# ArnaudPel/CamKifu

Hardware: AMD Instinct MI355X
Metric: frames/sec on 1920x1080 video + 19x19 stone-grid match % vs reference SGF (higher is better)
Workload: dtype u8+f16x2(f32 accumulate); 1 GPU; 1920x1080 synthetic game film, 256-frame batches resident in HBM, K1-K12 per ...; cnn=f16x2, frames_per_gpu=256, height=1080, width=1920, parallelism=frames of one video dealt x1, lanes_per_gpu=2, batches_in_flight=2

## Files before the change

### camkifu_amd/capi.py

```python
import ctypes as C
import os
import subprocess

import numpy as np

_HERE = os.path.dirname(os.path.abspath(__file__))
SO_PATH = os.environ.get("CK_HIP_LIB") or os.path.join(_HERE, "libck_hip.so")
CSRC = os.path.join(_HERE, "csrc")

CK_HOST, CK_DEVICE = 0, 1
CK_CNN_FP32, CK_CNN_BF16, CK_CNN_F16X2, CK_CNN_F16Q8 = 0, 1, 2, 3
CK_CNN_DEFAULT = CK_CNN_F16X2
CK_BOARD_LINES, CK_BOARD_NO_CONTOUR, CK_BOARD_TOO_SMALL = 0, 1, 2

ZONE_LINES = 32

EXPORTS = [
    "ck_ctx_create", "ck_ctx_create_prio", "ck_ctx_destroy", "ck_ctx_destroy2", "ck_stream_wait", "ck_last_error", "ck_backend", "ck_version", "ck_stream",
    "ck_timing_enable", "ck_timing_reset", "ck_timing_get",
    "ck_median15", "ck_median", "ck_canny", "ck_goban_canny", "ck_board_edges", "ck_board_lines", "ck_board_detect",
    "ck_i420_to_bgr", "ck_pyr_down", "ck_i420_to_bgr_pyr", "ck_get_perspective_transform", "ck_warp_perspective",
    "ck_mog2_create", "ck_mog2_apply", "ck_mog2_destroy", "ck_mog2_get_state",
    "ck_cnn_set_weights", "ck_cnn_set_mode", "ck_cnn_predict", "ck_cnn_maps", "ck_stones_detect",
    "ck_train_create", "ck_train_destroy", "ck_train_step", "ck_train_grads", "ck_train_apply", "ck_train_get_weights",
    "ck_train_get_adam_state", "ck_train_handover",
    "ck_cnn_regions", "ck_stones_run", "ck_zone_counts", "ck_mog2_band_run",
    "ck_board_detect_records", "ck_cnn_regions_records",
    "ck_contour_stones", "ck_cluster_stones", "ck_rng_get", "ck_rng_set", "ck_contours_external", "ck_find_intersections", "ck_update_grid",
    "ck_ordered_hull", "ck_boardfold_create", "ck_boardfold_destroy", "ck_boardfold_reset", "ck_boardfold_step", "ck_boardfold_run", "ck_round10", "ck_round10_reference",
    "ck_policy_create", "ck_policy_destroy", "ck_policy_run", "ck_policy_run_records", "ck_policy_get_state", "ck_policy_set_state",
    "ck_policy_watch",
]

WEIGHT_ORDER = ("c1w", "c1b", "c2w", "c2b", "c3w", "c3b", "c4w", "c4b", "d1w", "d1b", "d2w", "d2b")
WEIGHT_SHAPES = dict(c1w=(5, 5, 3, 32), c1b=(32,), c2w=(5, 5, 32, 32), c2b=(32,),
                     c3w=(3, 3, 32, 90), c3b=(90,), c4w=(3, 3, 90, 90), c4b=(90,),
                     d1w=(3240, 160), d1b=(160,), d2w=(160, 81), d2b=(81,))

# ... 64 lines not shown
        L.ck_policy_set_state.argtypes = [C.c_void_p, C.c_void_p, C.c_int]
        L.ck_policy_watch.argtypes = [C.c_void_p, C.c_int, C.c_int, C.c_int, C.c_double, C.c_longlong]
        L.ck_cluster_stones.argtypes = ([C.c_void_p, C.c_void_p, C.c_int, C.c_int, C.c_int, C.c_int, C.c_void_p, C.c_void_p, C.c_void_p,
                                        C.c_int] + [C.c_void_p] * 5 + [C.c_longlong] + [C.c_void_p] * 3)
        L.ck_rng_get.argtypes = [C.c_void_p, C.c_void_p]
        L.ck_train_step.argtypes = ([C.c_void_p, C.c_int, C.c_void_p, C.c_void_p] + [C.c_int] * 5
                                    + [C.c_double, C.c_int, C.c_uint64, C.c_void_p])
        L.ck_train_grads.argtypes = ([C.c_void_p, C.c_int, C.c_void_p, C.c_void_p] + [C.c_int] * 5
                                     + [C.c_int, C.c_uint64, C.c_longlong] + [C.c_void_p] * 5)
        L.ck_train_apply.argtypes = [C.c_void_p, C.c_int, C.c_void_p, C.c_double]
        L.ck_rng_set.argtypes = [C.c_void_p, C.c_uint64]
        _lib = L
    return _lib


def _is_torch(a):
    return type(a).__module__.startswith("torch")


def pyr_shape(h, w, levels):
    h, w, levels = int(h), int(w), int(levels)
    if levels < 0:
        raise CkError("pyramid levels %d: negative" % levels)
    for l in range(levels):
        if h < 2 or w < 2:
            raise CkError("pyramid level %d would take a %dx%d image: sides below 2" % (l + 1, w, h))
        h, w = (h + 1) // 2, (w + 1) // 2
    return h, w


# ... 265 lines not shown
    def cnn_set_weights(self, weights):
        ptrs = (C.c_void_p * 12)()
        keep, space = [], None
        for i, k in enumerate(WEIGHT_ORDER):
            a = weights[k]
            assert tuple(a.shape) == WEIGHT_SHAPES[k], (k, tuple(a.shape))
            if _is_torch(a):
                import torch
                assert a.dtype == torch.float32
            p, sp, ka = self._in(a, np.float32)
            assert space in (None, sp), "weights must live in one memory space"
            space = sp
            ptrs[i] = p
            keep.append(ka)
        self._chk(lib().ck_cnn_set_weights(self._h, ptrs, space))

    def cnn_set_mode(self, mode):
        self._chk(lib().ck_cnn_set_mode(self._h, int(mode)))

    def cnn_predict(self, goban, want_y=True):
        shp = tuple(goban.shape)
        n = 1 if len(shp) == 3 else shp[0]
        p, sp, keep = self._in(goban)
        y, yp = None, None
        if want_y:
            y, yp, _ = self._out(goban, (n, 100, 81), np.float32)
        labels, lp, osp = self._out(goban, (n, 19, 19), np.uint8)
        conf, cp, _ = self._out(goban, (n, 19, 19), np.float64)
        self._chk(lib().ck_cnn_predict(self._h, p, n, sp, yp, lp, cp, osp))
        return (y, labels, conf) if want_y else (labels, conf)
# ... 452 lines not shown
```

### camkifu_amd/csrc/ck_api.hip

```cpp
#include <stdarg.h>
#include <stddef.h>

#include <cfloat>
#include <cmath>
#include <algorithm>
#include <vector>
#include <thread>
#include <chrono>

#include "ck_common.h"
#include "ck_stonegeom.h"

thread_local std::string g_ck_create_error;
static thread_local const ck_ctx* g_ck_busy_ctx = nullptr;

unsigned long long ck_thread_token()
{
    static std::atomic<unsigned long long> next{1};
    static thread_local unsigned long long mine = 0;
    if (!mine) mine = next.fetch_add(1);
    return mine;
}
void ck_note_busy(const ck_ctx* ctx) { g_ck_busy_ctx = ctx; }

// ... 551 lines not shown
    return finish(ctx);
    CK_API_END(ctx)
}

int ck_cnn_set_weights(ck_ctx* ctx, const float* const weights[12], int space)
{
    CK_API_BEGIN(ctx)
    if (!ctx || !weights) return CK_ERR_ARG;
    for (int i = 0; i < 12; i++) if (!weights[i]) return ck_fail(ctx, CK_ERR_ARG, "weights[%d] is NULL", i);
    CK_HIP(ctx, hipSetDevice(ctx->device));
    CK_TRY(k_cnn_pack_weights(ctx, weights, space));
    return finish(ctx);
    CK_API_END(ctx)
}

int ck_cnn_set_mode(ck_ctx* ctx, int mode)
{
    CK_API_BEGIN(ctx)
    if (!ctx) return CK_ERR_ARG;
    if (mode != CK_CNN_FP32 && mode != CK_CNN_BF16 && mode != CK_CNN_F16X2 && mode != CK_CNN_F16Q8) return ck_fail(ctx, CK_ERR_ARG, "unknown cnn mode %d", mode);
    ctx->cnn_mode = mode;
    return CK_OK;
    CK_API_END(ctx)
}

struct RegionOut { uint8_t* label = nullptr; double* conf = nullptr; ck_frame_record* rec = nullptr; int rec_space = CK_HOST; };

static int ensure_rec_host(ck_ctx* ctx, size_t bytes)
{
    if (bytes <= ctx->rec_host_cap) return CK_OK;
// ... 620 lines not shown
```

### camkifu_amd/csrc/ck_common.h

```cpp
#pragma once
#include <hip/hip_runtime.h>
#include <stdint.h>
#include <stdio.h>
#include <string.h>
#include <atomic>
#include <condition_variable>
#include <functional>
#include <memory>
#include <mutex>
#include <exception>
#include <map>
#include <stdexcept>
#include <string>
#include <thread>
#include <vector>

#include "../../include/camkifu_amd.h"

struct DevBuf {
    void* p = nullptr;
    size_t cap = 0;
};

struct TimingSlot {
// ... 24 lines not shown
    long long steps = 0;
    DevBuf w, g, m, v;
    DevBuf lab, a1, a2, p1, a3, a4, p2, h1, lg, dlg, dh1, dp2, dz4, dz3, dp1, dz2, dz1, part, lossv, mask1, mask2, mask3;
};

static inline bool ck_cnn_split(int mode) { return mode == CK_CNN_F16X2 || mode == CK_CNN_F16Q8; }

struct CnnWeights {
    bool set = false;
    DevBuf c1w, c1b, c2w, c2b, c3w, c3b, c4w, c4b, d1w, d1b, d2w, d2b;
    DevBuf c2w_bf, c3w_bf, c4w_bf, d1w_bf;
    DevBuf c1w_f16;
    DevBuf d1w_bfp;
    DevBuf c1w_h2, c2w_h2, c3w_h2, c4w_h2, d1w_h2;
    DevBuf c1w_q8, c2x_q8, c3x_q8, c4x_q8;
    bool q8_ok = false;
};

struct ck_ctx {
    std::atomic<unsigned long long> owner{0};
    int depth = 0;
    int device = 0;
    hipStream_t stream = nullptr;
    std::string err;
    bool timing = false;
    std::map<std::string, TimingSlot> slots;
    std::vector<PendingEvent> pending;
    std::vector<hipEvent_t> event_pool;
    hipEvent_t handover = nullptr;

// ... 20 lines not shown
    DevBuf out_stage;
    DevBuf mats;
    DevBuf pyr0, pyr1;
    void* host_pinned = nullptr;
    size_t host_pinned_cap = 0;
    void* host_pinned2 = nullptr;
    size_t host_pinned2_cap = 0;
    void* rec_host = nullptr;
    size_t rec_host_cap = 0;
    DevBuf rec_stage;

    CnnWeights cnn;
    int* cnn_flag_host = nullptr;
    int* cnn_flag_dev = nullptr;
    int cnn_fallbacks = 0;
    int cnn_mode = CK_CNN_F16X2;
    std::vector<Mog2State> mog2;
    std::vector<CkTrainer> trainers;
    uint64_t rng_state = 0xffffffffULL;
};

extern thread_local std::string g_ck_create_error;

int ck_fail(ck_ctx* ctx, int code, const char* fmt, ...);
int ck_ensure(ck_ctx* ctx, DevBuf& b, size_t bytes);
int ck_ensure_pinned(ck_ctx* ctx, size_t bytes, int which = 0);

#define CK_HIP(ctx, call)                                                                 \
    do {                                                                                  \
        hipError_t e__ = (call);                                                          \
// ... 92 lines not shown
    std::vector<int32_t> pts;
};
int k_contour_survey(ck_ctx* ctx, const uint8_t* d_edges, int n, int h, int w, std::vector<std::vector<CkContour>>& out);
int ck_goban_canny_dev(ck_ctx* ctx, const uint8_t* d_in, int n, int h, int w, uint8_t* d_edges, double* otsu_out);
int k_contour_stones(ck_ctx* ctx, const uint8_t* d_goban, const uint8_t* d_fg, int n, int side, const int32_t* rects,
                     int rs, int re, int cs, int ce, uint8_t* stones, int16_t* zones_out, uint8_t* mask_out);
int k_cluster_stones(ck_ctx* ctx, const void* d_imgs, int n, int side, int is_f32, const int32_t* rects, const uint8_t* mask,
                     const int32_t* jobs, int m, uint8_t* stones, uint8_t* trusted, uint8_t* ratios, float* centers,
                     uint8_t* labels, long long labels_cap, int32_t* passes, double* compact, int32_t* winner);
double ck_otsu_level(const int* hist, size_t npx);
int k_grid_lines(ck_ctx* ctx, const uint8_t* d_goban, int n, int side, const int32_t* rects, const int16_t** lines_out,
                 const int32_t** nlines_out, uint8_t* edges_out);
int k_cnn_predict(ck_ctx* ctx, const uint8_t* d_goban, int n, float* d_y, uint8_t* d_labels, double* d_conf,
                  int* d_nonfinite = nullptr, uint8_t* d_rlabel = nullptr, double* d_rconf = nullptr);
int k_cnn_pack_weights(ck_ctx* ctx, const float* const w[12], int space);
int k_cnn_bf16_pack_conv1(ck_ctx* ctx, const float* k1, DevBuf& dst);
int k_cnn_bf16_convs(ck_ctx* ctx, const uint8_t* gob, int np, uint16_t* p2, uint16_t* q4);
int k_cnn_bf16_pack_fc1(ck_ctx* ctx, const float* w, DevBuf& dst);
int k_cnn_bf16_fc1(ck_ctx* ctx, const uint16_t* q4, int np, float* h1);
int k_cnn_q8_pack(ck_ctx* ctx, const float* k1, const float* k2, const float* k3, const float* k4);
int k_cnn_q8_conv12(ck_ctx* ctx, const uint8_t* gob, int np, float* p2, int* overflow);
int k_cnn_q8_conv34(ck_ctx* ctx, const float* p2, int np, float* p4, int* overflow);
extern const size_t CK_TRAIN_COUNTS[12];
size_t ck_train_offset(int i);
int k_train_create(ck_ctx* ctx, CkTrainer& tr, const float* const w[12], int space);
void k_train_free(CkTrainer& tr);
int k_train_grads(ck_ctx* ctx, CkTrainer& tr, const uint8_t* d_x, const uint8_t* d_lab, int n, int drop, uint64_t seed,
                  uint64_t step, bool want_masks);
int k_train_adam(ck_ctx* ctx, CkTrainer& tr, const float* d_g, double lr);
int k_mog2_apply(ck_ctx* ctx, Mog2State& st, const uint8_t* d_img, double lr, uint8_t* d_fg);
// ... 11 lines not shown
```

### camkifu_amd/csrc/k_cnn.hip

```cpp
#include <math.h>

#include <algorithm>

#include <type_traits>

#include "ck_common.h"

#ifndef C3_WM
#define C3_WM 2
#endif
#ifndef C4_WM
#define C4_WM 2
#endif
#ifndef H2_STAGE_UNROLL
#define H2_STAGE_UNROLL 8
#endif
#ifndef H2C2S_PF
#define H2C2S_PF 1
#endif
#ifndef H2C2S_SB
#define H2C2S_SB true
#endif
#ifndef H2C3_PF
#define H2C3_PF 2
// ... 36 lines not shown
__device__ unsigned long long g_h2_prof[8];
__device__ unsigned long long g_h34_prof[8];
constexpr int H2_LOG_CAP = 1 << 18;
__device__ unsigned long long g_h2_log[3 * H2_LOG_CAP];
#define H34_STAMP(K) do { if (NXT_W > 0 && threadIdx.x == 0) { const unsigned long long now__ = wall_clock64(); atomicAdd(&g_h34_prof[K], now__ - t_prev__); t_prev__ = now__; } } while (0)
#define H2_STAMP(K) do { if (FUSE1 && threadIdx.x == 0) { const unsigned long long now__ = wall_clock64(); atomicAdd(&g_h2_prof[K], now__ - t_prev__); t_prev__ = now__; } } while (0)
#else
#define H2_STAMP(K) do { } while (0)
#define H34_STAMP(K) do { } while (0)
#endif
#ifndef H2C34_RN
#define H2C34_RN 3
#endif
#ifndef H2C34_MINW
#define H2C34_MINW 2
#endif
#ifndef H2_C1_U
#define H2_C1_U 1
#endif
#ifndef H2C2S_WM
#define H2C2S_WM 8
#endif

namespace {

typedef float f32x16 __attribute__((ext_vector_type(16)));

__host__ __device__ constexpr int cdiv(int a, int b) { return (a + b - 1) / b; }

__host__ __device__ __forceinline__ uint16_t f2bf(float f)
{
    union { float f; uint32_t u; } x;
    x.f = f;
// ... 288 lines not shown
    hi = (_Float16)x;
    lo = (_Float16)(x - (float)hi);
}

typedef _Float16 h2v __attribute__((ext_vector_type(2)));
__device__ __forceinline__ void split_h2x2(float a, float b, h2v& hi, h2v& lo)
{
    const uint32_t hu = __builtin_bit_cast(uint32_t, __builtin_amdgcn_cvt_pkrtz(a, b));
    float ra, rb;
    asm("v_fma_mix_f32 %0, %1, -1.0, %2 op_sel_hi:[1,0,0]" : "=v"(ra) : "v"(hu), "v"(a));
    asm("v_fma_mix_f32 %0, %1, -1.0, %2 op_sel:[1,0,0] op_sel_hi:[1,0,0]" : "=v"(rb) : "v"(hu), "v"(b));
    hi = __builtin_bit_cast(h2v, hu);
    lo = __builtin_bit_cast(h2v, __builtin_amdgcn_cvt_pkrtz(ra, rb));
}

template <int CINP, bool POOL>
constexpr int h2_pspad() { return POOL ? (CINP == 96 ? 0 : 8) : (CINP == 32 ? 48 : 8); }
template <int CINP, bool POOL, int OW>
constexpr int h2_rsrem() { return POOL ? (CINP == 96 ? 16 : 32) : (CINP == 32 ? 32 : (8 * OW) % 64); }

constexpr int H2_IN1_HALVES = 21 * 128;
template <int H, int W, int CIN, int KH, int KW, int TB, bool POOL, bool SWZ>
constexpr int h2_tile_halves()
{
    constexpr int OW = W - KW + 1, M = (H - KH + 1) * OW, CINP = cdiv(CIN, 32) * 32;
    constexpr int PS = SWZ ? 2 * CINP : 2 * CINP + h2_pspad<CINP, POOL>();
    constexpr int RS = SWZ ? W * PS : lds_stride_b(W * PS, h2_rsrem<CINP, POOL, OW>(), 64);
    constexpr int ROWS_RAW = POOL ? 4 * (TB / (OW / 4)) + KH - 1 : (TB * 16 + OW - 2) / OW + 1 + KH - 1;
    (void)M;
    return (ROWS_RAW < H ? ROWS_RAW : H) * RS;
}

template <int H, int W, int CIN, int KH, int KW, int COUT, int TB, int YB, int WAVES_M, int RN, bool POOL, int PF, bool SB, bool FUSE1 = false,
          bool IN_LDS = false, int NXT_W = 0, int NXT_PS = 0, int NXT_RS = 0, int NXT_CINP = 0>
__device__ __forceinline__ void conv_h2_body(
    _Float16* __restrict__ lds, const int patch, const int blk_y,
    const float* __restrict__ in, const uint16_t* __restrict__ wt, const float* __restrict__ bias,
    float* __restrict__ out, float wscale_inv, int* __restrict__ overflow,
    const uint8_t* __restrict__ goban1 = nullptr, const uint16_t* __restrict__ wf1 = nullptr, const float* __restrict__ bias1 = nullptr)
{
#pragma clang fp contract(off)
    constexpr int OH = H - KH + 1, OW = W - KW + 1, M = OH * OW;
    constexpr int NT = cdiv(COUT, 16), WAVES_N = NT / RN;
    constexpr int CINP = cdiv(CIN, 32) * 32;
    static_assert(!FUSE1 || (CINP == 32 && POOL), "swizzled layout: 32 channels, pooling tiles");
    constexpr int PS = FUSE1 ? 2 * CINP : 2 * CINP + h2_pspad<CINP, POOL>();
    constexpr int RS = FUSE1 ? W * PS : lds_stride_b(W * PS, h2_rsrem<CINP, POOL, OW>(), 64);
    constexpr int KS = KH * KW * (CINP / 32);
    constexpr int NTHREADS = 64 * WAVES_M * WAVES_N;
// ... 26 lines not shown
        __shared__ __attribute__((aligned(16))) _Float16 in1[(IROWS + 1) * IRS];
        auto stage_pixels = [&](int p_, int by_, _Float16* dst) {
            const int oy_s = 4 * ((by_ * TB) / (OW / 4));
            int rows_s = H - oy_s;
            if (rows_s > ROWS) rows_s = ROWS;
            const int frame = p_ / 100, reg = p_ % 100;
            const int py0 = region_origin(reg / 10) + oy_s, px0 = region_origin(reg % 10);
            const int rows_in = rows_s + 4;
            const uint8_t* src = goban1 + ((size_t)frame * 380 + py0) * 380 * 3 + (size_t)px0 * 3;
            for (int d = tid; d < IROWS * 32 + IRS / 4; d += NTHREADS) {
                const int r = d >> 5, cd = d & 31;
                uint32_t raw = 0u;
                if (r < rows_in && cd < 30) raw = reinterpret_cast<const uint32_t*>(src + (size_t)r * 380 * 3)[cd];
                typedef _Float16 h4v __attribute__((ext_vector_type(4)));
                *reinterpret_cast<h4v*>(&dst[4 * d]) = h4v{(_Float16)(float)(raw & 0xFFu), (_Float16)(float)((raw >> 8) & 0xFFu),
                                                           (_Float16)(float)((raw >> 16) & 0xFFu), (_Float16)(float)(raw >> 24)};
            }
        };
        stage_pixels(patch, blk_y, in1);
        h8 w1[3][2][2];
#pragma unroll
        for (int sx = 0; sx < 3; sx++)
#pragma unroll
            for (int n = 0; n < 2; n++)
#pragma unroll
                for (int pl = 0; pl < 2; pl++)
                    w1[sx][n][pl] = __builtin_bit_cast(h8, reinterpret_cast<const uint4*>(wf1)[((n * 3 + sx) * 2 + pl) * 64 + lane]);
        float4 bv1[2];
#pragma unroll
        for (int n = 0; n < 2; n++) bv1[n] = *reinterpret_cast<const float4*>(bias1 + n * 16 + 4 * kq);
        __syncthreads();
        H2_STAMP(0);
        const int ntile1 = row_cnt * W / 16;
        constexpr int NW = NTHREADS / 64, R1 = cdiv(ROWS * W / 16, NW);
        float big = 0.f;
        auto conv1_tiles = [&](auto u_tag, int t_first) {
            constexpr int U = decltype(u_tag)::value;
            int a0[U], my[U], mx[U];
            uint32_t ash[U];
            f32x4 c1[U][2];
#pragma unroll
            for (int u = 0; u < U; u++) {
                const int m = (t_first + NW * u) * 16 + l15;
                my[u] = m / W; mx[u] = m % W;
                a0[u] = (my[u] + (kq >> 1)) * IRS + mx[u] * 3 + 8 * (kq & 1);
                ash[u] = (uint32_t)(a0[u] & 1) << 4;
#pragma unroll
                for (int n = 0; n < 2; n++) {
                    c1[u][n][0] = bv1[n].x * H2_WSCALE; c1[u][n][1] = bv1[n].y * H2_WSCALE;
                    c1[u][n][2] = bv1[n].z * H2_WSCALE; c1[u][n][3] = bv1[n].w * H2_WSCALE;
                }
            }
#pragma unroll
            for (int sx = 0; sx < 3; sx++) {
                h8 a[U];
#pragma unroll
                for (int u = 0; u < U; u++) {
                    const uint32_t* aq = reinterpret_cast<const uint32_t*>(&in1[(a0[u] & ~1) + 2 * sx * IRS]);
                    const uint32_t d0 = aq[0], d1 = aq[1], d2 = aq[2], d3 = aq[3], d4 = aq[4];
                    const uint4 au = make_uint4(__builtin_amdgcn_alignbit(d1, d0, ash[u]), __builtin_amdgcn_alignbit(d2, d1, ash[u]),
                                                __builtin_amdgcn_alignbit(d3, d2, ash[u]), __builtin_amdgcn_alignbit(d4, d3, ash[u]));
                    a[u] = __builtin_bit_cast(h8, au);
                }
#pragma unroll
                for (int n = 0; n < 2; n++) {
#pragma unroll
                    for (int u = 0; u < U; u++) c1[u][n] = __builtin_amdgcn_mfma_f32_16x16x32_f16(w1[sx][n][1], a[u], c1[u][n], 0, 0, 0);
#pragma unroll
                    for (int u = 0; u < U; u++) c1[u][n] = __builtin_amdgcn_mfma_f32_16x16x32_f16(w1[sx][n][0], a[u], c1[u][n], 0, 0, 0);
                }
            }
#pragma unroll
            for (int n = 0; n < 2; n++)
#pragma unroll
                for (int u = 0; u < U; u++) {
                    float v[4];
#pragma unroll
                    for (int e = 0; e < 4; e++) {
                        v[e] = c1[u][n][e] * wscale_inv;
                        v[e] = v[e] > 0.f ? v[e] : 0.f;
                    }
                    big = fmaxf(big, fmaxf(fmaxf(v[0], v[1]), fmaxf(v[2], v[3])));
                    typedef _Float16 h4v __attribute__((ext_vector_type(4)));
                    h2v h01, l01, h23, l23;
                    split_h2x2(v[0], v[1], h01, l01);
                    split_h2x2(v[2], v[3], h23, l23);
                    const h4v hi = {h01[0], h01[1], h23[0], h23[1]}, lo = {l01[0], l01[1], l23[0], l23[1]};
                    const int sw = h2_swz(mx[u], my[u]), c = 2 * n + (kq >> 1);
                    _Float16* px = &lds[my[u] * RS + mx[u] * PS + 4 * (kq & 1)];
                    *reinterpret_cast<h4v*>(px + ((c ^ sw) << 3)) = hi;
                    *reinterpret_cast<h4v*>(px + ((c ^ sw ^ 4) << 3)) = lo;
                }
        };
        {
            constexpr int U = H2_C1_U;
            int r = 0;
            if (H2_DBG_SKIP != 2) {
                for (; r + U <= R1 && wave + NW * (r + U - 1) < ntile1; r += U) conv1_tiles(std::integral_constant<int, U>{}, wave + NW * r);
                for (; r < R1 && wave + NW * r < ntile1; r++) conv1_tiles(std::integral_constant<int, 1>{}, wave + NW * r);
            }
        }
        if (overflow && !(big <= 65000.f)) *overflow = 1;
        H2_STAMP(4);
    } else if constexpr (!IN_LDS) {
        const float2* g = reinterpret_cast<const float2*>(in + ((size_t)patch * H + oy_min) * W * CIN);
        float big = 0.f;
        const int n_pairs = row_cnt * W * (CIN / 2);
        for (int i0 = tid; i0 < n_pairs; i0 += H2_STAGE_UNROLL * NTHREADS) {
            float2 vv[H2_STAGE_UNROLL];
#pragma unroll
            for (int u = 0; u < H2_STAGE_UNROLL; u++) {
                const int i = i0 + u * NTHREADS;
                vv[u] = i < n_pairs ? g[i] : make_float2(0.f, 0.f);
            }
#pragma unroll
            for (int u = 0; u < H2_STAGE_UNROLL; u++) {
                const int i = i0 + u * NTHREADS;
// ... 249 lines not shown
    if (FUSE1 && lane == 0) {
        unsigned hwid, xcc;
        asm volatile("s_getreg_b32 %0, hwreg(HW_REG_HW_ID)" : "=s"(hwid));
        asm volatile("s_getreg_b32 %0, hwreg(HW_REG_XCC_ID)" : "=s"(xcc));
        const unsigned wgid = patch * YB + blk_y;
        const unsigned slot = wgid * (NTHREADS / 64) + wave;
        if (slot < (unsigned)H2_LOG_CAP) {
            g_h2_log[3 * slot] = ((unsigned long long)wgid << 16) | ((xcc & 0xFu) << 8) | ((hwid >> 8) & 0xFFu);
            g_h2_log[3 * slot + 1] = t_born__;
            g_h2_log[3 * slot + 2] = wall_clock64();
        }
    }
#endif
}

template <int H, int W, int CIN, int KH, int KW, int COUT, int TB, int YB, int WAVES_M, int RN, bool POOL, int PF, bool SB, bool FUSE1>
__global__ __launch_bounds__(64 * WAVES_M * (cdiv(COUT, 16) / RN), (64 * WAVES_M * (cdiv(COUT, 16) / RN) >= 512 ? 4 : 1)) void conv_mfma16_h2_kernel(
    const float* __restrict__ in, const uint16_t* __restrict__ wt, const float* __restrict__ bias,
    float* __restrict__ out, float wscale_inv, int* __restrict__ overflow,
    const uint8_t* __restrict__ goban1 = nullptr, const uint16_t* __restrict__ wf1 = nullptr, const float* __restrict__ bias1 = nullptr)
{
    __shared__ __attribute__((aligned(16))) _Float16 lds[h2_tile_halves<H, W, CIN, KH, KW, TB, POOL, FUSE1>()];
    conv_h2_body<H, W, CIN, KH, KW, COUT, TB, YB, WAVES_M, RN, POOL, PF, SB, FUSE1>(lds, blockIdx.x, blockIdx.y, in, wt, bias, out,
                                                                                  wscale_inv, overflow, goban1, wf1, bias1);
}

__global__ __launch_bounds__(64 * 2 * (6 / H2C34_RN), H2C34_MINW) void conv34_h2_kernel(
    const float* __restrict__ in, const uint16_t* __restrict__ wt3, const float* __restrict__ bias3,
    const uint16_t* __restrict__ wt4, const float* __restrict__ bias4, float* __restrict__ out, float wscale_inv,
    int* __restrict__ overflow)
{
    constexpr int T3 = h2_tile_halves<16, 16, 32, 3, 3, 13, false, false>(), T4 = h2_tile_halves<14, 14, 90, 3, 3, 9, true, false>();
    constexpr int PS4 = 2 * 96 + h2_pspad<96, true>(), RS4 = lds_stride_b(14 * PS4, h2_rsrem<96, true, 12>(), 64);
    __shared__ __attribute__((aligned(16))) _Float16 lds[T3 > T4 ? T3 : T4];
#if H2_DBG_TIME
    const unsigned long long t0__ = wall_clock64();
#endif
    conv_h2_body<16, 16, 32, 3, 3, 90, 13, 1, 2, H2C34_RN, false, H2C3_PF, H2C3_SB, false, false, 14, PS4, RS4, 96>(
// ... 321 lines not shown
                if (kk >= 75) continue;
                const int i = kk / 15, j = (kk % 15) / 3, c = kk % 3;
                dst[((size_t)n * 19 + s) * 64 + lane] = k[(((size_t)(4 - i) * 5 + (4 - j)) * 3 + c) * 32 + o];
            }
}

static void pack_fc1(const float* w, std::vector<float>& dst)
{
    const int KIN = 3240, NOUT = 160, SG2 = KIN / 8;
    dst.assign((size_t)(NOUT / 16) * SG2 * 64 * 2, 0.f);
    for (int nt = 0; nt < NOUT / 16; nt++)
        for (int step = 0; step < KIN / 4; step++)
            for (int lane = 0; lane < 64; lane++)
                dst[(((size_t)nt * SG2 + step / 2) * 64 + lane) * 2 + step % 2] =
                    w[(size_t)(4 * step + lane / 16) * NOUT + nt * 16 + lane % 16];
}

int k_cnn_pack_weights(ck_ctx* ctx, const float* const w[12], int space)
{
    static const size_t counts[12] = { 5 * 5 * 3 * 32, 32, 5 * 5 * 32 * 32, 32, 3 * 3 * 32 * 90, 90,
                                       3 * 3 * 90 * 90, 90, 3240 * 160, 160, 160 * 81, 81 };
    std::vector<std::vector<float>> host(12);
    for (int i = 0; i < 12; i++) {
        host[i].resize(counts[i]);
        if (space == CK_DEVICE) CK_HIP(ctx, hipMemcpy(host[i].data(), w[i], counts[i] * 4, hipMemcpyDeviceToHost));
        else if (space == CK_HOST) memcpy(host[i].data(), w[i], counts[i] * 4);
        else return ck_fail(ctx, CK_ERR_ARG, "bad memory space %d", space);
    }
    auto up = [&](DevBuf& b, const std::vector<float>& v) -> int {
        CK_TRY(ck_ensure(ctx, b, v.size() * 4));
// ... 86 lines not shown
            for (int st = 0; st < 104; st++)
                for (int lane = 0; lane < 64; lane++)
                    for (int e = 0; e < 8; e++) {
                        const int k = 32 * st + 8 * (lane / 16) + e, o = 16 * t + lane % 16;
                        if (k >= 3240) continue;
                        const float wv = host[8][(size_t)k * 160 + o] * H2_WSCALE;
                        const _Float16 hi = (_Float16)wv;
                        const _Float16 lo = (_Float16)(wv - (float)hi);
                        const size_t base = (((size_t)t * 104 + st) * 2) * 64 * 8 + (size_t)lane * 8 + e;
                        memcpy(&v[base], &hi, 2);
                        memcpy(&v[base + 64 * 8], &lo, 2);
                    }
        CK_TRY(ck_ensure(ctx, ctx->cnn.d1w_h2, v.size() * 2));
        CK_HIP(ctx, hipMemcpy(ctx->cnn.d1w_h2.p, v.data(), v.size() * 2, hipMemcpyHostToDevice));
    }
    ctx->cnn.set = true;
    return CK_OK;
}

int k_cnn_predict(ck_ctx* ctx, const uint8_t* d_goban, int nframes, float* d_y, uint8_t* d_labels, double* d_conf,
                  int* d_nonfinite, uint8_t* d_rlabel, double* d_rconf)
{
    const int CHUNK = 128;
    const size_t a1_sz = (size_t)CHUNK * 100 * 36 * 36 * 32 * 4;
    const size_t p2_sz = (size_t)CHUNK * 100 * 12 * 12 * 90 * 4;
    CK_TRY(ck_ensure(ctx, ctx->act0, a1_sz));
    CK_TRY(ck_ensure(ctx, ctx->act1, p2_sz));
    CK_TRY(ck_ensure(ctx, ctx->act2, (size_t)nframes * 100 * (3240 + 160) * 4));
    float* a1 = (float*)ctx->act0.p;
    float* p2 = (float*)ctx->act1.p;
// ... 23 lines not shown
        const int nf = nframes - f0 < CHUNK ? nframes - f0 : CHUNK;
        const int np = nf * 100;
        const uint8_t* gob = d_goban + (size_t)f0 * 380 * 380 * 3;
        float* p4 = p4_all + (size_t)f0 * 100 * 3240;
        {
            TimeScope ts(ctx, "cnn_conv1");
            if (!q8 && !h2)
                hipLaunchKernelGGL((conv1_mfma16_kernel<C1_R>), dim3(std::min(np * 3, C1_GRID)), dim3(64 * (27 / C1_R)), 0,
                                   ctx->stream, gob, (const float*)W.c1w.p, (const float*)W.c1b.p, a1, np * 3);
        }
        {
            TimeScope ts(ctx, "cnn_conv2");
            if (q8) {
                CK_TRY(k_cnn_q8_conv12(ctx, gob, np, p2, d_nonfinite));
            } else if (h2) {
                hipLaunchKernelGGL((conv_mfma16_h2_kernel<36, 36, 32, 5, 5, 32, H2C2S_TB, 64 / H2C2S_TB + (64 % H2C2S_TB != 0), H2C2S_WM, 2, true, H2C2S_PF, H2C2S_SB, true>), dim3(np, 64 / H2C2S_TB + (64 % H2C2S_TB != 0)), dim3(64 * H2C2S_WM), 0, ctx->stream,
                                   (const float*)a1, (const uint16_t*)W.c2w_h2.p, (const float*)W.c2b.p, p2, 1.f / H2_WSCALE, d_nonfinite,
                                   gob, (const uint16_t*)W.c1w_h2.p, (const float*)W.c1b.p);
#if H2_DBG_TIME
                {
                    unsigned long long hp[8];
                    (void)hipStreamSynchronize(ctx->stream);
                    (void)hipMemcpyFromSymbol(hp, HIP_SYMBOL(g_h2_prof), sizeof hp);
                    if (hp[7]) fprintf(stderr, "[conv2 phases, us per workgroup over %llu workgroups] stage %.2f  conv1 tiles (wave 0) %.2f  wait for the others %.2f  k-loop %.2f  epilogue %.2f\n", hp[7],
                                       hp[0] * 0.01 / hp[7], hp[4] * 0.01 / hp[7], hp[1] * 0.01 / hp[7], hp[2] * 0.01 / hp[7], hp[3] * 0.01 / hp[7]);
                    memset(hp, 0, sizeof hp);
                    (void)hipMemcpyToSymbol(HIP_SYMBOL(g_h2_prof), hp, sizeof hp);
                    const int nw = std::min(np * 3 * 8, H2_LOG_CAP);
                    std::vector<unsigned long long> lg((size_t)3 * nw);
                    (void)hipMemcpyFromSymbol(lg.data(), HIP_SYMBOL(g_h2_log), lg.size() * 8);
                    struct Wg { unsigned long long a, b, wsum; int n; };
                    std::map<unsigned, std::map<unsigned, Wg>> cus;
                    unsigned long long t_lo = ~0ull, t_hi = 0;
// ... 95 lines not shown
```

### include/camkifu_amd.h

```cpp
#ifndef CAMKIFU_AMD_H
#define CAMKIFU_AMD_H

#include <stdint.h>

#ifdef __cplusplus
extern "C" {
#endif

enum { CK_OK = 0, CK_ERR_ARG = 1, CK_ERR_HIP = 2, CK_ERR_CAPACITY = 3, CK_ERR_STATE = 4 };
enum { CK_HOST = 0, CK_DEVICE = 1 };
enum { CK_BACKEND_HIP = 1 };
enum { CK_CNN_FP32 = 0, CK_CNN_BF16 = 1, CK_CNN_F16X2 = 2, CK_CNN_F16Q8 = 3 };

enum { CK_BOARD_LINES = 0,
       CK_BOARD_NO_CONTOUR = 1,
       CK_BOARD_TOO_SMALL = 2 };

typedef struct ck_ctx ck_ctx;

typedef struct ck_board_result {
    int32_t status;
    int32_t n_contours;
    int32_t n_lines;
    int32_t reserved;
// ... 44 lines not shown

int ck_get_perspective_transform(const float* src4, const float* dst4, double* M9);

int ck_warp_perspective(ck_ctx* ctx, const uint8_t* bgr, int n, int h, int w, int in_space,
                        const double* M, int m_count, int dsize,
                        uint8_t* out, int out_space);

int ck_mog2_create(ck_ctx* ctx, int h, int w, int* handle);
int ck_mog2_apply(ck_ctx* ctx, int handle, const uint8_t* img3, int in_space,
                  double learning_rate, uint8_t* fgmask, int out_space);
int ck_mog2_destroy(ck_ctx* ctx, int handle);
int ck_mog2_get_state(ck_ctx* ctx, int handle, float* weight, float* variance, float* mean, uint8_t* nmodes);

int ck_cnn_set_weights(ck_ctx* ctx, const float* const weights[12], int space);
int ck_cnn_set_mode(ck_ctx* ctx, int mode);
int ck_cnn_predict(ck_ctx* ctx, const uint8_t* goban, int n, int in_space,
                   float* y, uint8_t* labels, double* conf, int out_space);
int ck_cnn_maps(ck_ctx* ctx, const uint8_t* goban, int n, int in_space, float* pool2, float* pool4);

int ck_train_create(ck_ctx* ctx, const float* const weights[12], int space, int* handle);
int ck_train_destroy(ck_ctx* ctx, int handle);
int ck_train_step(ck_ctx* ctx, int handle, const uint8_t* x, const uint8_t* labels, int n, int h, int w, int c, int in_space,
                  double lr, int dropout, uint64_t seed, float* loss);
int ck_train_grads(ck_ctx* ctx, int handle, const uint8_t* x, const uint8_t* labels, int n, int h, int w, int c, int in_space,
                   int dropout, uint64_t seed, long long step, float* loss, float* const grads[12],
                   uint8_t* mask1, uint8_t* mask2, uint8_t* mask3);
int ck_train_apply(ck_ctx* ctx, int handle, const float* const grads[12], double lr);
int ck_train_get_weights(ck_ctx* ctx, int handle, float* const weights[12]);
int ck_train_get_adam_state(ck_ctx* ctx, int handle, float* const m[12], float* const v[12], long long* steps);
int ck_train_handover(ck_ctx* ctx, int handle);
// ... 90 lines not shown
```

Measured before the change: 23670 frames/s.

## Streamline fused conv1 loop and skip overflow watch when weights bound it

The fused conv1 stage in the f16x2 conv1+conv2 kernel is rewritten. It now walks one tile at a time with incrementally advanced read and store pointers instead of recomputing the index math per tile, and it drops the unroll knob. The input scale is folded into pixel staging, so the accumulator no longer needs a rescale before ReLU. ReLU and the max tracking run on integer bit patterns. On the host, a worst-case bound on the conv1 output is computed from the weights, and when it stays below the f16 overflow limit a kernel variant without the overflow check is launched. Counters and a bound-query API are added. The risk is small numeric differences from scaling the inputs before the MMA rather than after.

```diff
diff --git a/camkifu_amd/capi.py b/camkifu_amd/capi.py
--- a/camkifu_amd/capi.py
+++ b/camkifu_amd/capi.py
@@ -22,6 +22,7 @@
     "ck_i420_to_bgr", "ck_pyr_down", "ck_i420_to_bgr_pyr", "ck_get_perspective_transform", "ck_warp_perspective",
     "ck_mog2_create", "ck_mog2_apply", "ck_mog2_destroy", "ck_mog2_get_state",
     "ck_cnn_set_weights", "ck_cnn_set_mode", "ck_cnn_predict", "ck_cnn_maps", "ck_stones_detect",
+    "ck_cnn_conv1_bound", "ck_cnn_counters",
     "ck_train_create", "ck_train_destroy", "ck_train_step", "ck_train_grads", "ck_train_apply", "ck_train_get_weights",
     "ck_train_get_adam_state", "ck_train_handover",
     "ck_cnn_regions", "ck_stones_run", "ck_zone_counts", "ck_mog2_band_run",
@@ -116,6 +117,17 @@
     return _lib
 
 
+def cnn_conv1_bound(c1w, c1b):
+    w = np.ascontiguousarray(c1w, np.float32)
+    b = np.ascontiguousarray(c1b, np.float32)
+    assert w.shape == WEIGHT_SHAPES["c1w"] and b.shape == WEIGHT_SHAPES["c1b"], (w.shape, b.shape)
+    out = np.empty(32, np.float64)
+    rc = lib().ck_cnn_conv1_bound(w.ctypes.data_as(C.c_void_p), b.ctypes.data_as(C.c_void_p), out.ctypes.data_as(C.c_void_p))
+    if rc != 0:
+        raise CkError("ck_cnn_conv1_bound: error %d" % rc)
+    return out
+
+
 def _is_torch(a):
     return type(a).__module__.startswith("torch")
 
@@ -411,6 +423,11 @@
             ptrs[i] = p
             keep.append(ka)
         self._chk(lib().ck_cnn_set_weights(self._h, ptrs, space))
+
+    def cnn_counters(self):
+        c = (C.c_longlong * 3)()
+        self._chk(lib().ck_cnn_counters(self._h, c))
+        return dict(fallbacks=int(c[0]), conv12_unwatched=int(c[1]), conv12_watched=int(c[2]))
 
     def cnn_set_mode(self, mode):
         self._chk(lib().ck_cnn_set_mode(self._h, int(mode)))
diff --git a/camkifu_amd/csrc/ck_api.hip b/camkifu_amd/csrc/ck_api.hip
--- a/camkifu_amd/csrc/ck_api.hip
+++ b/camkifu_amd/csrc/ck_api.hip
@@ -589,6 +589,24 @@
     CK_API_END(ctx)
 }
 
+int ck_cnn_conv1_bound(const float* c1w, const float* c1b, double bound[32])
+{
+    if (!c1w || !c1b || !bound) return CK_ERR_ARG;
+    k_cnn_conv1_bound(c1w, c1b, bound);
+    return CK_OK;
+}
+
+int ck_cnn_counters(ck_ctx* ctx, long long counters[3])
+{
+    CK_API_BEGIN(ctx)
+    if (!ctx || !counters) return CK_ERR_ARG;
+    counters[0] = ctx->cnn_fallbacks;
+    counters[1] = ctx->cnn_c12_launches[0];
+    counters[2] = ctx->cnn_c12_launches[1];
+    return CK_OK;
+    CK_API_END(ctx)
+}
+
 int ck_cnn_set_mode(ck_ctx* ctx, int mode)
 {
     CK_API_BEGIN(ctx)
diff --git a/camkifu_amd/csrc/ck_common.h b/camkifu_amd/csrc/ck_common.h
--- a/camkifu_amd/csrc/ck_common.h
+++ b/camkifu_amd/csrc/ck_common.h
@@ -62,6 +62,7 @@
     DevBuf d1w_bfp;
     DevBuf c1w_h2, c2w_h2, c3w_h2, c4w_h2, d1w_h2;
     DevBuf c1w_q8, c2x_q8, c3x_q8, c4x_q8;
+    bool c1_watch = true;
     bool q8_ok = false;
 };
 
@@ -112,6 +113,7 @@
     int* cnn_flag_host = nullptr;
     int* cnn_flag_dev = nullptr;
     int cnn_fallbacks = 0;
+    long long cnn_c12_launches[2] = {0, 0};
     int cnn_mode = CK_CNN_F16X2;
     std::vector<Mog2State> mog2;
     std::vector<CkTrainer> trainers;
@@ -234,6 +236,7 @@
 int k_cnn_predict(ck_ctx* ctx, const uint8_t* d_goban, int n, float* d_y, uint8_t* d_labels, double* d_conf,
                   int* d_nonfinite = nullptr, uint8_t* d_rlabel = nullptr, double* d_rconf = nullptr);
 int k_cnn_pack_weights(ck_ctx* ctx, const float* const w[12], int space);
+double k_cnn_conv1_bound(const float* c1w, const float* c1b, double per_channel[32]);
 int k_cnn_bf16_pack_conv1(ck_ctx* ctx, const float* k1, DevBuf& dst);
 int k_cnn_bf16_convs(ck_ctx* ctx, const uint8_t* gob, int np, uint16_t* p2, uint16_t* q4);
 int k_cnn_bf16_pack_fc1(ck_ctx* ctx, const float* w, DevBuf& dst);
diff --git a/camkifu_amd/csrc/k_cnn.hip b/camkifu_amd/csrc/k_cnn.hip
--- a/camkifu_amd/csrc/k_cnn.hip
+++ b/camkifu_amd/csrc/k_cnn.hip
@@ -74,9 +74,6 @@
 #endif
 #ifndef H2C34_MINW
 #define H2C34_MINW 2
-#endif
-#ifndef H2_C1_U
-#define H2_C1_U 1
 #endif
 #ifndef H2C2S_WM
 #define H2C2S_WM 8
@@ -395,6 +392,12 @@
     lo = __builtin_bit_cast(h2v, __builtin_amdgcn_cvt_pkrtz(ra, rb));
 }
 
+__device__ __forceinline__ int relu_bits(float x)
+{
+    const int b = __builtin_bit_cast(int, x);
+    return b > 0 ? b : 0;
+}
+
 template <int CINP, bool POOL>
 constexpr int h2_pspad() { return POOL ? (CINP == 96 ? 0 : 8) : (CINP == 32 ? 48 : 8); }
 template <int CINP, bool POOL, int OW>
@@ -413,7 +416,7 @@
 }
 
 template <int H, int W, int CIN, int KH, int KW, int COUT, int TB, int YB, int WAVES_M, int RN, bool POOL, int PF, bool SB, bool FUSE1 = false,
-          bool IN_LDS = false, int NXT_W = 0, int NXT_PS = 0, int NXT_RS = 0, int NXT_CINP = 0>
+          bool IN_LDS = false, int NXT_W = 0, int NXT_PS = 0, int NXT_RS = 0, int NXT_CINP = 0, bool WATCH1 = true>
 __device__ __forceinline__ void conv_h2_body(
     _Float16* __restrict__ lds, const int patch, const int blk_y,
     const float* __restrict__ in, const uint16_t* __restrict__ wt, const float* __restrict__ bias,
@@ -470,7 +473,8 @@
                 if (r < rows_in && cd < 30) raw = reinterpret_cast<const uint32_t*>(src + (size_t)r * 380 * 3)[cd];
                 typedef _Float16 h4v __attribute__((ext_vector_type(4)));
                 *reinterpret_cast<h4v*>(&dst[4 * d]) = h4v{(_Float16)(float)(raw & 0xFFu), (_Float16)(float)((raw >> 8) & 0xFFu),
-                                                           (_Float16)(float)((raw >> 16) & 0xFFu), (_Float16)(float)(raw >> 24)};
+                                                           (_Float16)(float)((raw >> 16) & 0xFFu), (_Float16)(float)(raw >> 24)}
+                                                       * (_Float16)(1.f / H2_WSCALE);
             }
         };
         stage_pixels(patch, blk_y, in1);
@@ -488,75 +492,60 @@
         __syncthreads();
         H2_STAMP(0);
         const int ntile1 = row_cnt * W / 16;
-        constexpr int NW = NTHREADS / 64, R1 = cdiv(ROWS * W / 16, NW);
-        float big = 0.f;
-        auto conv1_tiles = [&](auto u_tag, int t_first) {
-            constexpr int U = decltype(u_tag)::value;
-            int a0[U], my[U], mx[U];
-            uint32_t ash[U];
-            f32x4 c1[U][2];
-#pragma unroll
-            for (int u = 0; u < U; u++) {
-                const int m = (t_first + NW * u) * 16 + l15;
-                my[u] = m / W; mx[u] = m % W;
-                a0[u] = (my[u] + (kq >> 1)) * IRS + mx[u] * 3 + 8 * (kq & 1);
-                ash[u] = (uint32_t)(a0[u] & 1) << 4;
+        constexpr int NW = NTHREADS / 64;
+        int big = 0;
+        constexpr int DY = NW * 16 / W, DX = NW * 16 % W;
+        static_assert(W % 2 == 0 && DX % 2 == 0, "a lane's columns keep their parity");
+        static_assert((DX & 7) == ((DY & 1) << 2) && ((DX - W) & 7) == (((DY + 1) & 1) << 2), "a lane's swizzle is the same for all its tiles");
+        static_assert(RS == W * PS && PS == 64, "a pixel's place in the swizzled tile is linear in its index");
+        const int wave_u = __builtin_amdgcn_readfirstlane(wave);
+        const int m0 = wave_u * 16 + l15;
+        int mx = m0 % W;
+        const int my0 = m0 / W;
+        const uint32_t ash = (uint32_t)(mx & 1) << 4;
+        const char* rd = reinterpret_cast<const char*>(in1) + 2 * (((my0 + (kq >> 1)) * IRS + mx * 3 + 8 * (kq & 1)) & ~1);
+        uint32_t st = 2 * (m0 * PS + 4 * (kq & 1) + (((kq >> 1) ^ h2_swz(mx, my0)) << 3));
+        char* const tile = reinterpret_cast<char*>(lds);
+        for (int t = wave_u; t < ntile1 && H2_DBG_SKIP != 2; t += NW) {
+            f32x4 c1[2] = {f32x4{bv1[0].x, bv1[0].y, bv1[0].z, bv1[0].w}, f32x4{bv1[1].x, bv1[1].y, bv1[1].z, bv1[1].w}};
+#pragma unroll
+            for (int sx = 0; sx < 3; sx++) {
+                const uint32_t* aq = reinterpret_cast<const uint32_t*>(rd + 2 * (2 * sx * IRS));
+                const uint32_t d0 = aq[0], d1 = aq[1], d2 = aq[2], d3 = aq[3], d4 = aq[4];
+                const uint4 au = make_uint4(__builtin_amdgcn_alignbit(d1, d0, ash), __builtin_amdgcn_alignbit(d2, d1, ash),
+                                            __builtin_amdgcn_alignbit(d3, d2, ash), __builtin_amdgcn_alignbit(d4, d3, ash));
+                const h8 a = __builtin_bit_cast(h8, au);
 #pragma unroll
                 for (int n = 0; n < 2; n++) {
-                    c1[u][n][0] = bv1[n].x * H2_WSCALE; c1[u][n][1] = bv1[n].y * H2_WSCALE;
-                    c1[u][n][2] = bv1[n].z * H2_WSCALE; c1[u][n][3] = bv1[n].w * H2_WSCALE;
+                    c1[n] = __builtin_amdgcn_mfma_f32_16x16x32_f16(w1[sx][n][1], a, c1[n], 0, 0, 0);
+                    c1[n] = __builtin_amdgcn_mfma_f32_16x16x32_f16(w1[sx][n][0], a, c1[n], 0, 0, 0);
                 }
             }
 #pragma unroll
-            for (int sx = 0; sx < 3; sx++) {
-                h8 a[U];
-#pragma unroll
-                for (int u = 0; u < U; u++) {
-                    const uint32_t* aq = reinterpret_cast<const uint32_t*>(&in1[(a0[u] & ~1) + 2 * sx * IRS]);
-                    const uint32_t d0 = aq[0], d1 = aq[1], d2 = aq[2], d3 = aq[3], d4 = aq[4];
-                    const uint4 au = make_uint4(__builtin_amdgcn_alignbit(d1, d0, ash[u]), __builtin_amdgcn_alignbit(d2, d1, ash[u]),
-                                                __builtin_amdgcn_alignbit(d3, d2, ash[u]), __builtin_amdgcn_alignbit(d4, d3, ash[u]));
-                    a[u] = __builtin_bit_cast(h8, au);
+            for (int n = 0; n < 2; n++) {
+                float v[4];
+                int vb[4];
+#pragma unroll
+                for (int e = 0; e < 4; e++) {
+                    vb[e] = relu_bits(c1[n][e]);
+                    v[e] = __builtin_bit_cast(float, vb[e]);
                 }
-#pragma unroll
-                for (int n = 0; n < 2; n++) {
-#pragma unroll
-                    for (int u = 0; u < U; u++) c1[u][n] = __builtin_amdgcn_mfma_f32_16x16x32_f16(w1[sx][n][1], a[u], c1[u][n], 0, 0, 0);
-#pragma unroll
-                    for (int u = 0; u < U; u++) c1[u][n] = __builtin_amdgcn_mfma_f32_16x16x32_f16(w1[sx][n][0], a[u], c1[u][n], 0, 0, 0);
-                }
-            }
-#pragma unroll
-            for (int n = 0; n < 2; n++)
-#pragma unroll
-                for (int u = 0; u < U; u++) {
-                    float v[4];
-#pragma unroll
-                    for (int e = 0; e < 4; e++) {
-                        v[e] = c1[u][n][e] * wscale_inv;
-                        v[e] = v[e] > 0.f ? v[e] : 0.f;
-                    }
-                    big = fmaxf(big, fmaxf(fmaxf(v[0], v[1]), fmaxf(v[2], v[3])));
-                    typedef _Float16 h4v __attribute__((ext_vector_type(4)));
-                    h2v h01, l01, h23, l23;
-                    split_h2x2(v[0], v[1], h01, l01);
-                    split_h2x2(v[2], v[3], h23, l23);
-                    const h4v hi = {h01[0], h01[1], h23[0], h23[1]}, lo = {l01[0], l01[1], l23[0], l23[1]};
-                    const int sw = h2_swz(mx[u], my[u]), c = 2 * n + (kq >> 1);
-                    _Float16* px = &lds[my[u] * RS + mx[u] * PS + 4 * (kq & 1)];
-                    *reinterpret_cast<h4v*>(px + ((c ^ sw) << 3)) = hi;
-                    *reinterpret_cast<h4v*>(px + ((c ^ sw ^ 4) << 3)) = lo;
-                }
-        };
-        {
-            constexpr int U = H2_C1_U;
-            int r = 0;
-            if (H2_DBG_SKIP != 2) {
-                for (; r + U <= R1 && wave + NW * (r + U - 1) < ntile1; r += U) conv1_tiles(std::integral_constant<int, U>{}, wave + NW * r);
-                for (; r < R1 && wave + NW * r < ntile1; r++) conv1_tiles(std::integral_constant<int, 1>{}, wave + NW * r);
-            }
-        }
-        if (overflow && !(big <= 65000.f)) *overflow = 1;
+                if constexpr (WATCH1) big = std::max(std::max(big, vb[0]), std::max(std::max(vb[1], vb[2]), vb[3]));
+                typedef _Float16 h4v __attribute__((ext_vector_type(4)));
+                h2v h01, l01, h23, l23;
+                split_h2x2(v[0], v[1], h01, l01);
+                split_h2x2(v[2], v[3], h23, l23);
+                const h4v hi = {h01[0], h01[1], h23[0], h23[1]}, lo = {l01[0], l01[1], l23[0], l23[1]};
+                *reinterpret_cast<h4v*>(tile + (st ^ (n << 5))) = hi;
+                *reinterpret_cast<h4v*>(tile + (st ^ (n << 5) ^ 64)) = lo;
+            }
+            mx += DX;
+            const bool wrap = mx >= W;
+            mx -= wrap ? W : 0;
+            rd += 2 * (wrap ? (DY + 1) * IRS + (DX - W) * 3 : DY * IRS + DX * 3);
+            st += 2 * NW * 16 * PS;
+        }
+        if (WATCH1 && overflow && big > __builtin_bit_cast(int, 65000.f)) *overflow = 1;
         H2_STAMP(4);
     } else if constexpr (!IN_LDS) {
         const float2* g = reinterpret_cast<const float2*>(in + ((size_t)patch * H + oy_min) * W * CIN);
@@ -836,14 +825,14 @@
 #endif
 }
 
-template <int H, int W, int CIN, int KH, int KW, int COUT, int TB, int YB, int WAVES_M, int RN, bool POOL, int PF, bool SB, bool FUSE1>
+template <int H, int W, int CIN, int KH, int KW, int COUT, int TB, int YB, int WAVES_M, int RN, bool POOL, int PF, bool SB, bool FUSE1, bool WATCH1>
 __global__ __launch_bounds__(64 * WAVES_M * (cdiv(COUT, 16) / RN), (64 * WAVES_M * (cdiv(COUT, 16) / RN) >= 512 ? 4 : 1)) void conv_mfma16_h2_kernel(
     const float* __restrict__ in, const uint16_t* __restrict__ wt, const float* __restrict__ bias,
     float* __restrict__ out, float wscale_inv, int* __restrict__ overflow,
     const uint8_t* __restrict__ goban1 = nullptr, const uint16_t* __restrict__ wf1 = nullptr, const float* __restrict__ bias1 = nullptr)
 {
     __shared__ __attribute__((aligned(16))) _Float16 lds[h2_tile_halves<H, W, CIN, KH, KW, TB, POOL, FUSE1>()];
-    conv_h2_body<H, W, CIN, KH, KW, COUT, TB, YB, WAVES_M, RN, POOL, PF, SB, FUSE1>(lds, blockIdx.x, blockIdx.y, in, wt, bias, out,
+    conv_h2_body<H, W, CIN, KH, KW, COUT, TB, YB, WAVES_M, RN, POOL, PF, SB, FUSE1, false, 0, 0, 0, 0, WATCH1>(lds, blockIdx.x, blockIdx.y, in, wt, bias, out,
                                                                                   wscale_inv, overflow, goban1, wf1, bias1);
 }
 
@@ -1195,6 +1184,19 @@
             for (int lane = 0; lane < 64; lane++)
                 dst[(((size_t)nt * SG2 + step / 2) * 64 + lane) * 2 + step % 2] =
                     w[(size_t)(4 * step + lane / 16) * NOUT + nt * 16 + lane % 16];
+}
+
+double k_cnn_conv1_bound(const float* c1w, const float* c1b, double per_channel[32])
+{
+    double worst = 0.0;
+    for (int o = 0; o < 32; o++) {
+        double sum = 0.0;
+        for (int k = 0; k < 75; k++) sum += fabs((double)c1w[(size_t)k * 32 + o]);
+        const double bound = fabs((double)c1b[o]) + 255.0 * sum;
+        if (per_channel) per_channel[o] = bound;
+        if (!(bound <= worst)) worst = bound;
+    }
+    return worst;
 }
 
 int k_cnn_pack_weights(ck_ctx* ctx, const float* const w[12], int space)
@@ -1311,6 +1313,7 @@
         CK_TRY(ck_ensure(ctx, ctx->cnn.d1w_h2, v.size() * 2));
         CK_HIP(ctx, hipMemcpy(ctx->cnn.d1w_h2.p, v.data(), v.size() * 2, hipMemcpyHostToDevice));
     }
+    ctx->cnn.c1_watch = !(k_cnn_conv1_bound(host[0].data(), host[1].data(), nullptr) <= 65000.0);
     ctx->cnn.set = true;
     return CK_OK;
 }
@@ -1364,9 +1367,16 @@
             if (q8) {
                 CK_TRY(k_cnn_q8_conv12(ctx, gob, np, p2, d_nonfinite));
             } else if (h2) {
-                hipLaunchKernelGGL((conv_mfma16_h2_kernel<36, 36, 32, 5, 5, 32, H2C2S_TB, 64 / H2C2S_TB + (64 % H2C2S_TB != 0), H2C2S_WM, 2, true, H2C2S_PF, H2C2S_SB, true>), dim3(np, 64 / H2C2S_TB + (64 % H2C2S_TB != 0)), dim3(64 * H2C2S_WM), 0, ctx->stream,
-                                   (const float*)a1, (const uint16_t*)W.c2w_h2.p, (const float*)W.c2b.p, p2, 1.f / H2_WSCALE, d_nonfinite,
-                                   gob, (const uint16_t*)W.c1w_h2.p, (const float*)W.c1b.p);
+                constexpr int YB2 = 64 / H2C2S_TB + (64 % H2C2S_TB != 0);
+                auto conv12 = [&](auto watch) {
+                    hipLaunchKernelGGL((conv_mfma16_h2_kernel<36, 36, 32, 5, 5, 32, H2C2S_TB, YB2, H2C2S_WM, 2, true, H2C2S_PF, H2C2S_SB, true, decltype(watch)::value>),
+                                       dim3(np, YB2), dim3(64 * H2C2S_WM), 0, ctx->stream,
+                                       (const float*)a1, (const uint16_t*)W.c2w_h2.p, (const float*)W.c2b.p, p2, 1.f / H2_WSCALE, d_nonfinite,
+                                       gob, (const uint16_t*)W.c1w_h2.p, (const float*)W.c1b.p);
+                };
+                if (W.c1_watch) conv12(std::true_type{});
+                else conv12(std::false_type{});
+                ctx->cnn_c12_launches[W.c1_watch ? 1 : 0]++;
 #if H2_DBG_TIME
                 {
                     unsigned long long hp[8];
diff --git a/include/camkifu_amd.h b/include/camkifu_amd.h
--- a/include/camkifu_amd.h
+++ b/include/camkifu_amd.h
@@ -82,6 +82,8 @@
 
 int ck_cnn_set_weights(ck_ctx* ctx, const float* const weights[12], int space);
 int ck_cnn_set_mode(ck_ctx* ctx, int mode);
+int ck_cnn_conv1_bound(const float* c1w, const float* c1b, double bound[32]);
+int ck_cnn_counters(ck_ctx* ctx, long long counters[3]);
 int ck_cnn_predict(ck_ctx* ctx, const uint8_t* goban, int n, int in_space,
                    float* y, uint8_t* labels, double* conf, int out_space);
 int ck_cnn_maps(ck_ctx* ctx, const uint8_t* goban, int n, int in_space, float* pool2, float* pool4);
```

Measured after the change: 23320 frames/s. 0.985x the previous value.
